# gk969/stm32-speech-recognition

Hardware: AMD Instinct MI355X
Metric: utterances/sec (256-frame, 100 templates) (higher is better)
Workload: dtype int32

## Files before the change

### stm32_speech_recognition_amd/csrc/k_mfcc.hip

```cpp
#include "sr_fft_dev.h"

#ifndef SR_MEL_CHUNKED
#define SR_MEL_CHUNKED 1
#endif

namespace sr {

constexpr int kMfccWaves = 4;
constexpr int kFramesPerWave = 16, kFramesPerWaveMid = 4, kFramesPerWaveSmall = 1;
constexpr int kMelPad = kMel + 1;
__device__ __forceinline__ constexpr int mel_chunk_word(int j) { return 256 * ((j >> 2) & 1) + 4 * ((j >> 3) ^ (4 * ((j >> 2) & 1))) + (j & 3); }
constexpr int mfcc_wave_lds_words(int fpw) { return kXchgWords + fpw * kMelPad + 64; }

template <int kFPW, typename Args = MfccArgs>
__global__ void __launch_bounds__(64 * kMfccWaves, 4) k_mfcc(const Args a)
{
    constexpr int kFeat = mfcc_feat_kind<Args>;
    constexpr uint32_t kFeatW = (kFeat == SR_FEAT_FFT || kFeat == SR_FEAT_MAG) ? kBins : kMel;
    constexpr int kWaveLdsWords = mfcc_wave_lds_words(kFPW);
    extern __shared__ __attribute__((aligned(16))) uint32_t smem[];
    __shared__ uint32_t s_dctM[kCoef * kMelPad];
    __shared__ int s_dctS[kCoef * kMelPad];
    __shared__ u32x4 s_tw3[kTw3Row * 4], s_tw5[8 * 64];
    __shared__ u32x4 s_tm[4 * 64];
    const int lane = threadIdx.x & 63, w = __builtin_amdgcn_readfirstlane(threadIdx.x >> 6);
    uint32_t *buf = smem + w * kWaveLdsWords;
    uint32_t *xw = buf;
    uint32_t *powb = buf + kXchgWords, *moff = powb + kFPW * kMelPad;

    for (int i = threadIdx.x; i < kCoef * kMel; i += blockDim.x) {
        const int c = a.t.dct[i], o = (i / kMel) * kMelPad + i % kMel;
        s_dctM[o] = (uint32_t)(((c < 0 ? -c : c) * 262144 + 99) / 100);
        s_dctS[o] = (c > 0) - (c < 0);
    }
    __syncthreads();

    LaneTw tw;
    load_lane_tw(a.t, lane, tw);
    if (w == 0 && lane < 4) {
        const uint32_t *f = &tw.s3[0][0][0];
#pragma unroll
        for (int c = 0; c < 8; c++) s_tw3[lane * kTw3Row + c] = u32x4{f[4 * c], f[4 * c + 1], f[4 * c + 2], f[4 * c + 3]};
    }
    if (w == 1 % kMfccWaves) store_tw32(s_tw5, lane, tw.s5);
#ifndef SR_INJECT_LDS_RACE
    if (w == 2 % kMfccWaves) {
#pragma unroll
        for (int c = 0; c < 2; c++) {
            s_tm[64 * c + lane] = *(const u32x4 *)(a.t.tri_even_m + 8 * lane + 4 * c);
            s_tm[64 * (c + 2) + lane] = *(const u32x4 *)(a.t.tri_odd_m + 8 * lane + 4 * c);
        }
    }
#endif
    __syncthreads();
#ifdef SR_INJECT_LDS_RACE
    if (w == 2 % kMfccWaves) {
#if SR_INJECT_LDS_RACE >= 2
        __builtin_amdgcn_s_sleep(127);
#endif
#pragma unroll
        for (int c = 0; c < 2; c++) {
            s_tm[64 * c + lane] = *(const u32x4 *)(a.t.tri_even_m + 8 * lane + 4 * c);
            s_tm[64 * (c + 2) + lane] = *(const u32x4 *)(a.t.tri_odd_m + 8 * lane + 4 * c);
        }
    }
#endif
    int hamm_m[3];
#pragma unroll
    for (int k = 0; k < 3; k++) hamm_m[k] = (lane + 64 * k < kFrameLen) ? hamm_fused_multiplier(a.t.hamm[lane + 64 * k]) : 0;
    int f_lo = 0, p_hi = 0, p_lo = 0, x_hi = 0, x_lo = 0;
    if (lane < kMel) {
        const int h = lane;
        f_lo = (h == 0) ? 0 : (int)a.t.tri_cen[h - 1];
        const int f_hi = (h == kMel - 1) ? kBins : (int)a.t.tri_cen[h + 1];
        const int ih = f_hi - 1, il = f_lo ? f_lo - 1 : 0, half = (h & 1) ? kBins : 0;
#if SR_MEL_CHUNKED
        p_hi = half + mel_chunk_word(ih), x_hi = (ih >> 3) > 0 ? (ih >> 3) - 1 : 0;
        p_lo = half + mel_chunk_word(il), x_lo = (il >> 3) > 0 ? (il >> 3) - 1 : 0;
#else
        p_hi = half + ih, x_hi = (ih >> 3) > 0 ? (ih >> 3) - 1 : 0;
        p_lo = half + il, x_lo = (il >> 3) > 0 ? (il >> 3) - 1 : 0;
#endif
    }
    const uint32_t tw_off = 32u * (uint32_t)lane;
#if SR_MEL_CHUNKED
    const int e_base = mel_chunk_word(lane);
    constexpr int kEs = 32, kEh = 128;
    const int c0 = mel_chunk_word(8 * lane), c1 = mel_chunk_word(8 * lane + 4);
#else
    const int e_base = lane;
    constexpr int kEs = 64, kEh = 256;
    const int c0 = 8 * lane, c1 = 8 * lane + 4;
#endif

    uint32_t item = blockIdx.x;
    uint32_t nx_nfrm = 0;
    int nx_mid = 0, nx_seg0 = 0;
    if (item < a.n_items) {
        const sr_vad_rec *rec = a.vad + item / a.tiles;
        nx_nfrm = rec->frm_num;
        nx_mid = (int)rec->atap.mid_val;
        nx_seg0 = rec->seg[0];
    }
    for (; item < a.n_items; item += gridDim.x) {
        const uint32_t b = item / a.tiles, tile = item - b * a.tiles;
        const uint32_t nfrm = nx_nfrm;
        const int mid = nx_mid, seg0 = nx_seg0;
        if (item + gridDim.x < a.n_items) {
            const sr_vad_rec *rec = a.vad + (item + gridDim.x) / a.tiles;
            nx_nfrm = rec->frm_num;
            nx_mid = (int)rec->atap.mid_val;
            nx_seg0 = rec->seg[0];
        }
        const uint16_t *row = a.pcm + (uint64_t)b * a.pcm_stride;
        int16_t *out = a.mfcc + (uint64_t)b * a.max_frames * kCoef;
        const uint32_t f0 = tile * (kMfccWaves * kFPW) + w * kFPW;
        uint32_t *frow = nullptr;
        if constexpr (kFeat != 0) frow = a.feat + (uint64_t)b * a.max_frames * kFeatW;
        uint32_t nf = 0;
        if (f0 < nfrm) nf = (nfrm - f0 < (uint32_t)kFPW) ? nfrm - f0 : (uint32_t)kFPW;

        uint32_t s_pp[3] = {0, 0, 0};
        if (nf) {
            const uint16_t *x = row + seg0 + (int)kHop * (int)f0;
#pragma unroll
            for (int k = 0; k < 3; k++) {
                const int i = lane + 64 * k;
                if (i < kFrameLen) s_pp[k] = *(const u32_align2 *)(x + i - 1);
            }
        }
        for (uint32_t fi = 0; fi < nf; fi++) {
#pragma unroll
            for (int k = 0; k < 3; k++) {
                const int i = lane + 64 * k;
                if (i < kFrameLen) xw[i] = k == 0 ? window_sample<4>(s_pp[k], mid, hamm_m[k]) : window_sample<2>(s_pp[k], mid, hamm_m[k]);
            }
            if (fi + 1 < nf) {
                const uint16_t *x = row + seg0 + (int)kHop * (int)(f0 + fi + 1);
#pragma unroll
                for (int k = 0; k < 3; k++) {
                    const int i = lane + 64 * k;
                    if (i < kFrameLen) s_pp[k] = *(const u32_align2 *)(x + i - 1);
                }
            }
            wave_sync();
            uint32_t v[4][4], u[4][4];
            fft_front_real160(xw, lane, tw, s_tw3, v);
            fft_exchange(buf, lane, v, u);
#pragma unroll
            for (int e4 = 0; e4 < 4; e4++)
                bfly_pk<false>(u[0][e4], u[1][e4], u[2][e4], u[3][e4], tw.s4[0][0], tw.s4[0][1], tw.s4[1][0], tw.s4[1][1],
                               tw.s4[2][0], tw.s4[2][1], tw.s4[3][0], tw.s4[3][1]);
            wave_sync();
            uint32_t k5[4][4][2];
            load_tw32(s_tw5, lane, k5);
            uint32_t nn[8];
#pragma unroll
            for (int e3 = 0; e3 < 4; e3++) {
                bfly_pk<true>(u[e3][0], u[e3][1], u[e3][2], u[e3][3], k5[e3][0][0], k5[e3][0][1], k5[e3][1][0],
                              k5[e3][1][1], k5[e3][2][0], k5[e3][2][1], k5[e3][3][0], k5[e3][3][1]);
                if constexpr (kFeat == SR_FEAT_FFT) {
                    uint32_t *fr = frow + (f0 + fi) * kFeatW + lane + 64 * e3;
                    fr[0] = u[e3][0];
                    fr[256] = u[e3][1];
                }
                nn[2 * e3] = (uint32_t)sdot2z(u[e3][0], u[e3][0]);
                nn[2 * e3 + 1] = (uint32_t)sdot2z(u[e3][1], u[e3][1]);
            }
            const uint32_t nmax = max(max(max(max(nn[0], nn[1]), nn[2]), max(max(nn[3], nn[4]), nn[5])), max(nn[6], nn[7]));
            const bool quiet = __builtin_expect(__builtin_amdgcn_ballot_w64(nmax > kMagSmallMax) == 0, 1);
            u32x4 tw_e[2], tw_o[2];
            bool cheap = true;
            if (!quiet) {
#pragma unroll
                for (int c = 0; c < 2; c++) {
                    tw_e[c] = *(const u32x4 *)((const char *)a.t.tri_even32 + tw_off + 16 * c);
                    tw_o[c] = *(const u32x4 *)((const char *)a.t.tri_odd32 + tw_off + 16 * c);
                }
                cheap = __builtin_amdgcn_ballot_w64(nmax > a.mag_cheap_max) == 0;
            } else {
                asm volatile("" : "=v"(tw_e[0]), "=v"(tw_e[1]), "=v"(tw_o[0]), "=v"(tw_o[1]));
            }
            uint32_t *eb = buf + e_base;
            if (cheap) {
#pragma unroll
                for (int e3 = 0; e3 < 4; e3++) {
                    const f32x2 m = f32x2{__builtin_amdgcn_sqrtf((float)(int)nn[2 * e3]), __builtin_amdgcn_sqrtf((float)(int)nn[2 * e3 + 1])} *
                                    f32x2{10.0f, 10.0f};
                    const uint32_t m0 = cvt_u32(m.x), m1 = cvt_u32(m.y);
                    if constexpr (kFeat == SR_FEAT_MAG) {
                        uint32_t *fr = frow + (f0 + fi) * kFeatW + lane + 64 * e3;
                        fr[0] = m0;
                        fr[256] = m1;
                    }
                    eb[kEs * e3] = umul24(m0, m0);
                    eb[kEs * e3 + kEh] = umul24(m1, m1);
                }
            } else {
#pragma unroll
                for (int e3 = 0; e3 < 4; e3++) {
                    const f32x2 m = sqrt_rn_int2(f32x2{(float)(int)nn[2 * e3], (float)(int)nn[2 * e3 + 1]}) * f32x2{10.0f, 10.0f};
                    const uint32_t m0 = cvt_u32(m.x), m1 = cvt_u32(m.y);
                    if constexpr (kFeat == SR_FEAT_MAG) {
                        uint32_t *fr = frow + (f0 + fi) * kFeatW + lane + 64 * e3;
                        fr[0] = m0;
                        fr[256] = m1;
                    }
                    eb[kEs * e3] = umul24(m0, m0);
                    eb[kEs * e3 + kEh] = umul24(m1, m1);
                }
            }
            wave_sync();
            uint32_t pe[8], po[8], xe, xo;
            {
                const uint4 q0 = *(const uint4 *)(buf + c0), q1 = *(const uint4 *)(buf + c1);
                const uint32_t e[8] = {q0.x, q0.y, q0.z, q0.w, q1.x, q1.y, q1.z, q1.w};
                uint32_t se = 0, so = 0;
                if (quiet) {
#pragma unroll
                    for (int c = 0; c < 2; c++) {
                        const u32x4 me = s_tm[64 * c + lane], mo = s_tm[64 * (c + 2) + lane];
#pragma unroll
                        for (int k = 0; k < 4; k++) {
                            const uint32_t es = e[4 * c + k] << 4;
                            se += mel_term_fused(es, me[k]);
                            so += mel_term_fused(es, mo[k]);
                            pe[4 * c + k] = se;
                            po[4 * c + k] = so;
                        }
                    }
                } else {
#pragma unroll
                    for (int c = 0; c < 2; c++) {
#pragma unroll
                        for (int k = 0; k < 4; k++) {
                            se += e[4 * c + k] * tw_e[c][k] / 100u;
                            so += e[4 * c + k] * tw_o[c][k] / 100u;
                            pe[4 * c + k] = se;
                            po[4 * c + k] = so;
                        }
                    }
                }
                xe = wave_scan_incl(se);
                xo = wave_scan_incl(so);
            }
            *(uint4 *)(buf + c0) = make_uint4(pe[0], pe[1], pe[2], pe[3]);
            *(uint4 *)(buf + c1) = make_uint4(pe[4], pe[5], pe[6], pe[7]);
            *(uint4 *)(buf + kBins + c0) = make_uint4(po[0], po[1], po[2], po[3]);
            *(uint4 *)(buf + kBins + c1) = make_uint4(po[4], po[5], po[6], po[7]);
            buf[2 * kBins + lane] = xe;
            moff[lane] = xo;
            wave_sync();
            if (lane < kMel) {
                const uint32_t *X = (lane & 1) ? moff : buf + 2 * kBins;
                const uint32_t hi = buf[p_hi] + X[x_hi], lo = f_lo ? buf[p_lo] + X[x_lo] : 0u;
                powb[fi * kMelPad + lane] = hi - lo;
                if constexpr (kFeat == SR_FEAT_MEL) frow[(f0 + fi) * kFeatW + lane] = hi - lo;
            }
            wave_sync();
        }

        {
            constexpr int kLogRounds = (kFPW * kMelPad + 63) / 64;
            const uint32_t n_log = nf * kMelPad;
            uint32_t nv[kLogRounds], mv[kLogRounds];
            u32x2 tv[kLogRounds];
#pragma unroll
            for (int r = 0; r < kLogRounds; r++) {
                const uint32_t t = lane + 64u * r;
                nv[r] = powb[t];
                mv[r] = log100_est(nv[r]);
                tv[r] = *(const u32_pair_align4 *)((const char *)a.t.log_thr + 4u * mv[r]);
            }
#pragma unroll
            for (int r = 0; r < kLogRounds; r++) {
                const uint32_t t = lane + 64u * r;
                if (t < n_log) powb[t] = log100_fix(nv[r], mv[r], tv[r].x, tv[r].y) << 14;
            }
        }
        wave_sync();
        if constexpr (kFeat == SR_FEAT_LOGMEL) {
            uint32_t *fw = frow + f0 * kFeatW;
            for (uint32_t t = lane; t < nf * kFeatW; t += 64) {
                const uint32_t fi = t / kFeatW, h = t - fi * kFeatW;
                fw[t] = powb[fi * kMelPad + h] >> 14;
            }
        }
        {
            int16_t *out_w = out + (size_t)f0 * kCoef;
#pragma unroll
            for (uint32_t t = lane; t < (uint32_t)(kFPW * kCoef); t += 64) {
                if (t < nf * kCoef) {
                    const uint32_t fi = umul24(t, 10923u) >> 17, h = t - umul24(fi, (uint32_t)kCoef);
                    const uint32_t *pw = powb + umul24(fi, (uint32_t)kMelPad), *dm = s_dctM + umul24(h, (uint32_t)kMelPad);
                    const int *ds = s_dctS + umul24(h, (uint32_t)kMelPad);
                    int acc = 0;
#pragma unroll
                    for (int i = 0; i < kMel; i++) acc = mad24((int)__umulhi(pw[i], dm[i]), ds[i], acc);
                    out_w[t] = (int16_t)acc;
                }
            }
        }
        wave_sync();
        {
            const uint32_t r0 = f0 + nf, r1 = (f0 + kFPW < a.max_frames) ? f0 + kFPW : a.max_frames;
            for (uint32_t t = r0 * kCoef + lane; t < r1 * kCoef && r0 < r1; t += 64) out[t] = 0;
        }
        if constexpr (kFeat != 0) {
            const uint32_t r0 = f0 + nf, r1 = (f0 + kFPW < a.max_frames) ? f0 + kFPW : a.max_frames;
            for (uint32_t t = r0 * kFeatW + lane; t < r1 * kFeatW && r0 < r1; t += 64) frow[t] = 0;
        }
    }
}

uint32_t mfcc_ext_frames_per_tile();
int mfcc_ext_occupancy(int *per_cu);
void launch_mfcc_ext(const MfccArgs &a, uint32_t grid, hipStream_t s);
void launch_mfcc_ext_features(const MfccArgs &a, int kind, uint32_t *feat, uint32_t grid, hipStream_t s);

uint32_t mfcc_frames_per_tile(uint32_t frame_len) { return frame_len == 320 ? mfcc_ext_frames_per_tile() : (uint32_t)(kMfccWaves * kFramesPerWave); }
uint32_t mfcc_frames_per_tile_small(uint32_t frame_len, uint32_t which)
{
    return frame_len == 320 ? mfcc_ext_frames_per_tile() : (uint32_t)(kMfccWaves * (which ? kFramesPerWaveSmall : kFramesPerWaveMid));
}

uint32_t mfcc_resident_workgroups(uint32_t frame_len)
{
    int dev = 0, n_cu = 0, per_cu = 0;
    if (hipGetDevice(&dev) != hipSuccess) return 0;
    if (hipDeviceGetAttribute(&n_cu, hipDeviceAttributeMultiprocessorCount, dev) != hipSuccess || n_cu < 1) return 0;
    int e;
    if (frame_len == 320)
        e = mfcc_ext_occupancy(&per_cu);
    else
        e = (int)hipOccupancyMaxActiveBlocksPerMultiprocessor(&per_cu, k_mfcc<kFramesPerWave>, 64 * kMfccWaves,
                                                              (size_t)kMfccWaves * mfcc_wave_lds_words(kFramesPerWave) * sizeof(uint32_t));
    if (e != (int)hipSuccess || per_cu < 1) return 0;
    return (uint32_t)(per_cu * n_cu);
}

void launch_mfcc(const MfccArgs &a, hipStream_t s)
{
    if (a.generic) {
        launch_mfcc_gen(a, s);
        return;
    }
    if (a.n_items == 0) return;
    const uint32_t cap = a.grid_cap ? a.grid_cap : 4096u;
    const uint32_t grid = a.n_items < cap ? a.n_items : cap;
    if (a.frame_len == 320) {
        launch_mfcc_ext(a, grid, s);
        return;
    }
    if (a.small_tiles == 2) {
        const size_t lds = (size_t)kMfccWaves * mfcc_wave_lds_words(kFramesPerWaveSmall) * sizeof(uint32_t);
        hipLaunchKernelGGL(k_mfcc<kFramesPerWaveSmall>, dim3(grid), dim3(64 * kMfccWaves), lds, s, a);
        return;
    }
    if (a.small_tiles == 1) {
        const size_t lds = (size_t)kMfccWaves * mfcc_wave_lds_words(kFramesPerWaveMid) * sizeof(uint32_t);
        hipLaunchKernelGGL(k_mfcc<kFramesPerWaveMid>, dim3(grid), dim3(64 * kMfccWaves), lds, s, a);
        return;
    }
    const size_t lds = (size_t)kMfccWaves * mfcc_wave_lds_words(kFramesPerWave) * sizeof(uint32_t);
    hipLaunchKernelGGL(k_mfcc<kFramesPerWave>, dim3(grid), dim3(64 * kMfccWaves), lds, s, a);
}

template <int kFPW, int kKind>
static void launch_mfcc_feat_kind(const MfccArgs &a, uint32_t *feat, uint32_t grid, hipStream_t s)
{
    const size_t lds = (size_t)kMfccWaves * mfcc_wave_lds_words(kFPW) * sizeof(uint32_t);
    hipLaunchKernelGGL((k_mfcc<kFPW, MfccFeatArgs<kKind>>), dim3(grid), dim3(64 * kMfccWaves), lds, s, mfcc_feat_args<kKind>(a, feat));
}
template <int kFPW>
static void launch_mfcc_feat_form(const MfccArgs &a, int kind, uint32_t *feat, uint32_t grid, hipStream_t s)
{
    switch (kind) {
    case SR_FEAT_FFT: launch_mfcc_feat_kind<kFPW, SR_FEAT_FFT>(a, feat, grid, s); break;
    case SR_FEAT_MAG: launch_mfcc_feat_kind<kFPW, SR_FEAT_MAG>(a, feat, grid, s); break;
    case SR_FEAT_MEL: launch_mfcc_feat_kind<kFPW, SR_FEAT_MEL>(a, feat, grid, s); break;
    case SR_FEAT_LOGMEL: launch_mfcc_feat_kind<kFPW, SR_FEAT_LOGMEL>(a, feat, grid, s); break;
    default: break;
    }
}

void launch_mfcc_features(const MfccArgs &a, int kind, uint32_t *feat, hipStream_t s)
{
    if (a.generic) {
        launch_mfcc_gen_features(a, kind, feat, s);
        return;
    }
    if (a.n_items == 0) return;
    const uint32_t cap = a.grid_cap ? a.grid_cap : 4096u;
    const uint32_t grid = a.n_items < cap ? a.n_items : cap;
    if (a.frame_len == 320)
        launch_mfcc_ext_features(a, kind, feat, grid, s);
    else if (a.small_tiles == 2)
        launch_mfcc_feat_form<kFramesPerWaveSmall>(a, kind, feat, grid, s);
    else if (a.small_tiles == 1)
        launch_mfcc_feat_form<kFramesPerWaveMid>(a, kind, feat, grid, s);
    else
        launch_mfcc_feat_form<kFramesPerWave>(a, kind, feat, grid, s);
}

}
```

### stm32_speech_recognition_amd/csrc/sr_dev.h

```cpp
#pragma once
#include <cstdlib>

#include "sr_device.h"
#include "sr_tables.h"

namespace sr {

typedef short short2v __attribute__((ext_vector_type(2)));
typedef uint32_t u32x2 __attribute__((ext_vector_type(2)));
typedef uint32_t u32x4 __attribute__((ext_vector_type(4)));

__device__ __forceinline__ int sdot2(uint32_t a, uint32_t b, int c)
{
    return __builtin_amdgcn_sdot2(__builtin_bit_cast(short2v, a), __builtin_bit_cast(short2v, b), c, false);
}
__device__ __forceinline__ int sext_lo(uint32_t w) { return (int)(short)(w & 0xFFFFu); }
__device__ __forceinline__ int sext_hi(uint32_t w) { return (int)w >> 16; }
__device__ __forceinline__ uint32_t pack16(int re, int im) { return ((uint32_t)re & 0xFFFFu) | ((uint32_t)im << 16); }

__device__ __forceinline__ int sdot2z(uint32_t a, uint32_t b)
{
    int r;
    asm("v_dot2_i32_i16 %0, %1, %2, 0" : "=v"(r) : "v"(a), "v"(b));
    return r;
}
__device__ __forceinline__ int sdot2a(uint32_t a, uint32_t b, int c)
{
    int r;
    asm("v_dot2_i32_i16 %0, %1, %2, %3" : "=v"(r) : "v"(a), "v"(b), "v"(c));
    return r;
}
__device__ __forceinline__ int preemph95(int p) { return (int)((float)p * 0.95000005f); }
__device__ __forceinline__ int neg_preemph95(int p) { return (int)((float)p * -0.95000005f); }
__device__ __forceinline__ int window_quotient(int c, int nq, int hm)
{
    int u;
    asm("v_add_lshl_u32 %0, %1, %2, %3" : "=v"(u) : "v"(c), "v"(nq), "n"(kWinShift));
    const long long P = (long long)u * (long long)hm + (long long)(unsigned long long)(uint32_t)(u >> 31);
    return (int)(P >> 32);
}
template <int SH = 2>
__device__ __forceinline__ uint32_t window_sample(uint32_t prev_cur, int mid, int hm)
{
    const int nq = neg_preemph95((int)(prev_cur & 0xFFFFu) - mid);
    const int c = (int)(prev_cur >> 16) - mid;
    int u;
    asm("v_add_lshl_u32 %0, %1, %2, %3" : "=v"(u) : "v"(c), "v"(nq), "n"(kWinShift));
    const long long P = (long long)u * (long long)hm + (long long)(unsigned long long)(uint32_t)(u >> 31);
    int r;
    asm("v_bfe_i32 %0, %1, %2, %3" : "=v"(r) : "v"((int)(P >> 32)), "n"(SH), "n"(16 - SH));
    return (uint32_t)r;
}
__device__ __forceinline__ int mul24(int a, int b) { return __mul24(a, b); }
__device__ __forceinline__ uint32_t umul24(uint32_t a, uint32_t b) { return __umul24(a, b); }
__device__ __forceinline__ int mad24(int a, int b, int c)
{
    int r;
    asm("v_mad_i32_i24 %0, %1, %2, %3" : "=v"(r) : "v"(a), "v"(b), "v"(c));
    return r;
}

__device__ __forceinline__ uint32_t mel_term_fused(uint32_t e_shl4, uint32_t m) { return __umulhi(e_shl4, m); }
__device__ __forceinline__ uint32_t mel_tri_of_multiplier(uint32_t m) { return __umulhi(m, 1600u); }

__device__ __forceinline__ float sqrt_rn_int(float f)
{
    const float y = __builtin_amdgcn_rsqf(f);
    const float s0 = f * y, h = 0.5f * y;
    const float r = __builtin_fmaf(-s0, s0, f);
    return __builtin_fmaf(r, h, s0);
}

__device__ __forceinline__ uint32_t mag10_small(float f)
{
    uint32_t r;
    const float m = __builtin_amdgcn_sqrtf(f) * 10.0f;
    asm("v_cvt_u32_f32 %0, %1" : "=v"(r) : "v"(m));
    return r;
}

__device__ __forceinline__ uint32_t cvt_u32(float x)
{
    uint32_t r;
    asm("v_cvt_u32_f32 %0, %1" : "=v"(r) : "v"(x));
    return r;
}
typedef float f32x2 __attribute__((ext_vector_type(2)));
__device__ __forceinline__ f32x2 sqrt_rn_int2(f32x2 f)
{
    const f32x2 y = {__builtin_amdgcn_rsqf(f.x), __builtin_amdgcn_rsqf(f.y)};
    const f32x2 s0 = f * y, h = f32x2{0.5f, 0.5f} * y;
    const f32x2 r = __builtin_elementwise_fma(-s0, s0, f);
    return __builtin_elementwise_fma(r, h, s0);
}
typedef uint32_t u32_align2 __attribute__((aligned(2)));
typedef uint32_t u32x2_raw __attribute__((ext_vector_type(2)));
typedef u32x2_raw u32_pair_align4 __attribute__((aligned(4)));
typedef uint32_t u32x2_align2 __attribute__((ext_vector_type(2), aligned(2)));

typedef unsigned short u16x2 __attribute__((ext_vector_type(2)));
__device__ __forceinline__ uint32_t pk_add(uint32_t a, uint32_t b)
{
    return __builtin_bit_cast(uint32_t, (u16x2)(__builtin_bit_cast(u16x2, a) + __builtin_bit_cast(u16x2, b)));
}
__device__ __forceinline__ uint32_t pk_sub(uint32_t a, uint32_t b)
{
    return __builtin_bit_cast(uint32_t, (u16x2)(__builtin_bit_cast(u16x2, a) - __builtin_bit_cast(u16x2, b)));
}
__device__ __forceinline__ uint32_t pk_ashr(uint32_t a, int n)
{
    return __builtin_bit_cast(uint32_t, (short2v)(__builtin_bit_cast(short2v, a) >> (short2v){(short)n, (short)n}));
}
__device__ __forceinline__ uint32_t pk_lshr(uint32_t a, int n)
{
    return __builtin_bit_cast(uint32_t, (u16x2)(__builtin_bit_cast(u16x2, a) >> (u16x2){(unsigned short)n, (unsigned short)n}));
}
__device__ __forceinline__ uint32_t pk_mad(uint32_t a, uint32_t c, uint32_t b)
{
    return __builtin_bit_cast(uint32_t, (u16x2)(__builtin_bit_cast(u16x2, a) * __builtin_bit_cast(u16x2, c) +
                                                __builtin_bit_cast(u16x2, b)));
}
__device__ __forceinline__ uint32_t pk_mad_swap(uint32_t a, uint32_t c, uint32_t b)
{
    uint32_t r;
    asm("v_pk_mad_u16 %0, %1, %2, %3 op_sel:[1,0,0] op_sel_hi:[0,1,1]" : "=v"(r) : "v"(a), "s"(c), "v"(b));
    return r;
}
__device__ __forceinline__ uint32_t pk_hi16(int lo_src, int hi_src)
{
    return __builtin_amdgcn_perm((uint32_t)hi_src, (uint32_t)lo_src, 0x07060302u);
}
__device__ __forceinline__ uint32_t pk_s15(int lo_src, int hi_src)
{
    uint32_t r = (uint32_t)lo_src >> 15;
    asm("v_lshrrev_b32_sdwa %0, %1, %2 dst_sel:WORD_1 dst_unused:UNUSED_PRESERVE src0_sel:DWORD src1_sel:DWORD\n\ts_nop 0"
        : "+v"(r)
        : "v"(15), "v"(hi_src));
    return r;
}

__device__ __forceinline__ void wave_sync()
{
    __builtin_amdgcn_fence(__ATOMIC_RELEASE, "wavefront");
    __builtin_amdgcn_wave_barrier();
    __builtin_amdgcn_fence(__ATOMIC_ACQUIRE, "wavefront");
}

__device__ __forceinline__ uint32_t wave_sum(uint32_t v)
{
#pragma unroll
    for (int d = 32; d >= 1; d >>= 1) v += __shfl_xor(v, d, 64);
    return v;
}
__device__ __forceinline__ uint32_t wave_min_u32(uint32_t v)
{
#pragma unroll
    for (int d = 32; d >= 1; d >>= 1) {
        uint32_t o = __shfl_xor(v, d, 64);
        v = o < v ? o : v;
    }
    return v;
}
__device__ __forceinline__ uint32_t wave_max(uint32_t v)
{
#pragma unroll
    for (int d = 32; d >= 1; d >>= 1) {
        uint32_t o = __shfl_xor(v, d, 64);
        v = o > v ? o : v;
    }
    return v;
}

template <int CTRL, int ROW_MASK>
__device__ __forceinline__ uint32_t dpp_take(uint32_t v)
{
    return (uint32_t)__builtin_amdgcn_update_dpp(0, (int)v, CTRL, ROW_MASK, 0xF, false);
}
__device__ __forceinline__ uint32_t wave_scan_incl(uint32_t v)
{
    v += dpp_take<0x111, 0xF>(v);
    v += dpp_take<0x112, 0xF>(v);
    v += dpp_take<0x114, 0xF>(v);
    v += dpp_take<0x118, 0xF>(v);
    asm("s_nop 1\n\tv_add_u32_dpp %0, %0, %0 row_bcast:15 row_mask:0xa" : "+v"(v));
    asm("s_nop 1\n\tv_add_u32_dpp %0, %0, %0 row_bcast:31 row_mask:0xc" : "+v"(v));
    return v;
}

__device__ __forceinline__ uint32_t log100_est(uint32_t n)
{
    return (uint32_t)(int)__builtin_amdgcn_fmed3f(__log2f((float)n) * 69.31471806f, 1.0f, (float)(kLogMax - 1));
}
__device__ __forceinline__ uint32_t log100_fix(uint32_t n, uint32_t m, uint32_t t0, uint32_t t1)
{
    return (uint32_t)((int)m - (int)(n < t0) + (int)(n >= t1));
}
__device__ __forceinline__ uint32_t log100_u32(uint32_t n, const uint32_t *__restrict__ thr)
{
    const uint32_t m = log100_est(n);
    return log100_fix(n, m, thr[m], thr[m + 1]);
}

}
```

Measured before the change: 3.172 million.

## Process frame pairs per wave, sharing overlapping PCM loads and pre-emphasis

For the 16-frames-per-wave variant, the loop now handles two consecutive frames per iteration. One set of global loads covers both frames' overlapping sample window. Pre-emphasis is computed once and staged through LDS, and each frame gets its own Hamming multiply. This cuts redundant global loads and pre-emphasis work for overlapping frames, at the cost of extra LDS traffic, a wave sync and more register pressure.

Result: no change. 3.183 million, median of 6 (+0.3%).

```diff
diff --git a/stm32_speech_recognition_amd/csrc/k_mfcc.hip b/stm32_speech_recognition_amd/csrc/k_mfcc.hip
--- a/stm32_speech_recognition_amd/csrc/k_mfcc.hip
+++ b/stm32_speech_recognition_amd/csrc/k_mfcc.hip
@@ -11,6 +11,10 @@
 constexpr int kMelPad = kMel + 1;
 __device__ __forceinline__ constexpr int mel_chunk_word(int j) { return 256 * ((j >> 2) & 1) + 4 * ((j >> 3) ^ (4 * ((j >> 2) & 1))) + (j & 3); }
 constexpr int mfcc_wave_lds_words(int fpw) { return kXchgWords + fpw * kMelPad + 64; }
+__device__ __forceinline__ bool pair_row_has(int k, int lane, bool two)
+{
+    return k < 2 || (k == 2 && (two || lane < kFrameLen - 128)) || (k == 3 && two && lane < kFrameLen + kHop - 192);
+}
 
 template <int kFPW, typename Args = MfccArgs>
 __global__ void __launch_bounds__(64 * kMfccWaves, 4) k_mfcc(const Args a)
@@ -68,6 +72,12 @@
     int hamm_m[3];
 #pragma unroll
     for (int k = 0; k < 3; k++) hamm_m[k] = (lane + 64 * k < kFrameLen) ? hamm_fused_multiplier(a.t.hamm[lane + 64 * k]) : 0;
+    constexpr bool kPair = kFPW == kFramesPerWave;
+    constexpr uint32_t kStep = kPair ? 2 : 1;
+    constexpr int kRows = kPair ? 4 : 3;
+    const int hamm_m2 = kPair ? hamm_fused_multiplier(a.t.hamm[128 + (lane & 31)]) : 0;
+    uint32_t *tpre = buf + 576 - kHop;
+    const int t2 = 128 + lane + (lane >= 32 ? kHop - 32 : 0);
     int f_lo = 0, p_hi = 0, p_lo = 0, x_hi = 0, x_lo = 0;
     if (lane < kMel) {
         const int h = lane;
@@ -120,144 +130,177 @@
         uint32_t nf = 0;
         if (f0 < nfrm) nf = (nfrm - f0 < (uint32_t)kFPW) ? nfrm - f0 : (uint32_t)kFPW;
 
-        uint32_t s_pp[3] = {0, 0, 0};
+        uint32_t s_pp[kRows] = {};
         if (nf) {
             const uint16_t *x = row + seg0 + (int)kHop * (int)f0;
-#pragma unroll
-            for (int k = 0; k < 3; k++) {
-                const int i = lane + 64 * k;
-                if (i < kFrameLen) s_pp[k] = *(const u32_align2 *)(x + i - 1);
-            }
-        }
-        for (uint32_t fi = 0; fi < nf; fi++) {
-#pragma unroll
-            for (int k = 0; k < 3; k++) {
-                const int i = lane + 64 * k;
-                if (i < kFrameLen) xw[i] = k == 0 ? window_sample<4>(s_pp[k], mid, hamm_m[k]) : window_sample<2>(s_pp[k], mid, hamm_m[k]);
-            }
-            if (fi + 1 < nf) {
-                const uint16_t *x = row + seg0 + (int)kHop * (int)(f0 + fi + 1);
+            const bool two = kPair && nf > 1;
+#pragma unroll
+            for (int k = 0; k < kRows; k++)
+                if (pair_row_has(k, lane, two)) s_pp[k] = *(const u32_align2 *)(x + lane + 64 * k - 1);
+        }
+        uint32_t hb0 = 0, hb1 = 0, h2 = 0;
+        for (uint32_t fi = 0; fi < nf; fi += kStep) {
+            if constexpr (kPair) {
+                int u[kRows];
+#pragma unroll
+                for (int k = 0; k < kRows; k++) u[k] = window_pre(s_pp[k], mid);
+#pragma unroll
+                for (int k = 1; k < kRows; k++) tpre[64 * k + lane] = (uint32_t)u[k];
+                xw[lane] = window_hamm<4>(u[0], hamm_m[0]);
+                xw[64 + lane] = window_hamm<2>(u[1], hamm_m[1]);
+                if (fi + 2 < nf) {
+                    const uint16_t *x = row + seg0 + (int)kHop * (int)(f0 + fi + 2);
+                    const bool two = fi + 3 < nf;
+#pragma unroll
+                    for (int k = 0; k < kRows; k++)
+                        if (pair_row_has(k, lane, two)) s_pp[k] = *(const u32_align2 *)(x + lane + 64 * k - 1);
+                }
+                wave_sync();
+                h2 = window_hamm<2>((int)tpre[t2], hamm_m2);
+                if (lane < 32) xw[128 + lane] = h2;
+                hb0 = window_hamm<4>((int)tpre[kHop + lane], hamm_m[0]);
+                hb1 = window_hamm<2>((int)tpre[kHop + 64 + lane], hamm_m[1]);
+            } else {
 #pragma unroll
                 for (int k = 0; k < 3; k++) {
                     const int i = lane + 64 * k;
-                    if (i < kFrameLen) s_pp[k] = *(const u32_align2 *)(x + i - 1);
+                    if (i < kFrameLen) xw[i] = k == 0 ? window_sample<4>(s_pp[k], mid, hamm_m[k]) : window_sample<2>(s_pp[k], mid, hamm_m[k]);
+                }
+                if (fi + 1 < nf) {
+                    const uint16_t *x = row + seg0 + (int)kHop * (int)(f0 + fi + 1);
+#pragma unroll
+                    for (int k = 0; k < 3; k++) {
+                        const int i = lane + 64 * k;
+                        if (i < kFrameLen) s_pp[k] = *(const u32_align2 *)(x + i - 1);
+                    }
                 }
             }
             wave_sync();
-            uint32_t v[4][4], u[4][4];
-            fft_front_real160(xw, lane, tw, s_tw3, v);
-            fft_exchange(buf, lane, v, u);
-#pragma unroll
-            for (int e4 = 0; e4 < 4; e4++)
-                bfly_pk<false>(u[0][e4], u[1][e4], u[2][e4], u[3][e4], tw.s4[0][0], tw.s4[0][1], tw.s4[1][0], tw.s4[1][1],
-                               tw.s4[2][0], tw.s4[2][1], tw.s4[3][0], tw.s4[3][1]);
-            wave_sync();
-            uint32_t k5[4][4][2];
-            load_tw32(s_tw5, lane, k5);
-            uint32_t nn[8];
-#pragma unroll
-            for (int e3 = 0; e3 < 4; e3++) {
-                bfly_pk<true>(u[e3][0], u[e3][1], u[e3][2], u[e3][3], k5[e3][0][0], k5[e3][0][1], k5[e3][1][0],
-                              k5[e3][1][1], k5[e3][2][0], k5[e3][2][1], k5[e3][3][0], k5[e3][3][1]);
-                if constexpr (kFeat == SR_FEAT_FFT) {
-                    uint32_t *fr = frow + (f0 + fi) * kFeatW + lane + 64 * e3;
-                    fr[0] = u[e3][0];
-                    fr[256] = u[e3][1];
-                }
-                nn[2 * e3] = (uint32_t)sdot2z(u[e3][0], u[e3][0]);
-                nn[2 * e3 + 1] = (uint32_t)sdot2z(u[e3][1], u[e3][1]);
-            }
-            const uint32_t nmax = max(max(max(max(nn[0], nn[1]), nn[2]), max(max(nn[3], nn[4]), nn[5])), max(nn[6], nn[7]));
-            const bool quiet = __builtin_expect(__builtin_amdgcn_ballot_w64(nmax > kMagSmallMax) == 0, 1);
-            u32x4 tw_e[2], tw_o[2];
-            bool cheap = true;
-            if (!quiet) {
-#pragma unroll
-                for (int c = 0; c < 2; c++) {
-                    tw_e[c] = *(const u32x4 *)((const char *)a.t.tri_even32 + tw_off + 16 * c);
-                    tw_o[c] = *(const u32x4 *)((const char *)a.t.tri_odd32 + tw_off + 16 * c);
-                }
-                cheap = __builtin_amdgcn_ballot_w64(nmax > a.mag_cheap_max) == 0;
-            } else {
-                asm volatile("" : "=v"(tw_e[0]), "=v"(tw_e[1]), "=v"(tw_o[0]), "=v"(tw_o[1]));
-            }
-            uint32_t *eb = buf + e_base;
-            if (cheap) {
+#pragma unroll
+            for (uint32_t s = 0; s < kStep; s++) {
+                const uint32_t fc = fi + s;
+                if (s == 1) {
+                    if (fc >= nf) break;
+                    xw[lane] = hb0;
+                    xw[64 + lane] = hb1;
+                    if (lane >= 32) xw[96 + lane] = h2;
+                    wave_sync();
+                }
+                uint32_t v[4][4], u[4][4];
+                fft_front_real160(xw, lane, tw, s_tw3, v);
+                fft_exchange(buf, lane, v, u);
+#pragma unroll
+                for (int e4 = 0; e4 < 4; e4++)
+                    bfly_pk<false>(u[0][e4], u[1][e4], u[2][e4], u[3][e4], tw.s4[0][0], tw.s4[0][1], tw.s4[1][0], tw.s4[1][1],
+                                   tw.s4[2][0], tw.s4[2][1], tw.s4[3][0], tw.s4[3][1]);
+                wave_sync();
+                uint32_t k5[4][4][2];
+                load_tw32(s_tw5, lane, k5);
+                uint32_t nn[8];
 #pragma unroll
                 for (int e3 = 0; e3 < 4; e3++) {
-                    const f32x2 m = f32x2{__builtin_amdgcn_sqrtf((float)(int)nn[2 * e3]), __builtin_amdgcn_sqrtf((float)(int)nn[2 * e3 + 1])} *
-                                    f32x2{10.0f, 10.0f};
-                    const uint32_t m0 = cvt_u32(m.x), m1 = cvt_u32(m.y);
-                    if constexpr (kFeat == SR_FEAT_MAG) {
-                        uint32_t *fr = frow + (f0 + fi) * kFeatW + lane + 64 * e3;
-                        fr[0] = m0;
-                        fr[256] = m1;
-                    }
-                    eb[kEs * e3] = umul24(m0, m0);
-                    eb[kEs * e3 + kEh] = umul24(m1, m1);
-                }
-            } else {
-#pragma unroll
-                for (int e3 = 0; e3 < 4; e3++) {
-                    const f32x2 m = sqrt_rn_int2(f32x2{(float)(int)nn[2 * e3], (float)(int)nn[2 * e3 + 1]}) * f32x2{10.0f, 10.0f};
-                    const uint32_t m0 = cvt_u32(m.x), m1 = cvt_u32(m.y);
-                    if constexpr (kFeat == SR_FEAT_MAG) {
-                        uint32_t *fr = frow + (f0 + fi) * kFeatW + lane + 64 * e3;
-                        fr[0] = m0;
-                        fr[256] = m1;
-                    }
-                    eb[kEs * e3] = umul24(m0, m0);
-                    eb[kEs * e3 + kEh] = umul24(m1, m1);
-                }
-            }
-            wave_sync();
-            uint32_t pe[8], po[8], xe, xo;
-            {
-                const uint4 q0 = *(const uint4 *)(buf + c0), q1 = *(const uint4 *)(buf + c1);
-                const uint32_t e[8] = {q0.x, q0.y, q0.z, q0.w, q1.x, q1.y, q1.z, q1.w};
-                uint32_t se = 0, so = 0;
-                if (quiet) {
+                    bfly_pk<true>(u[e3][0], u[e3][1], u[e3][2], u[e3][3], k5[e3][0][0], k5[e3][0][1], k5[e3][1][0],
+                                  k5[e3][1][1], k5[e3][2][0], k5[e3][2][1], k5[e3][3][0], k5[e3][3][1]);
+                    if constexpr (kFeat == SR_FEAT_FFT) {
+                        uint32_t *fr = frow + (f0 + fc) * kFeatW + lane + 64 * e3;
+                        fr[0] = u[e3][0];
+                        fr[256] = u[e3][1];
+                    }
+                    nn[2 * e3] = (uint32_t)sdot2z(u[e3][0], u[e3][0]);
+                    nn[2 * e3 + 1] = (uint32_t)sdot2z(u[e3][1], u[e3][1]);
+                }
+                const uint32_t nmax = max(max(max(max(nn[0], nn[1]), nn[2]), max(max(nn[3], nn[4]), nn[5])), max(nn[6], nn[7]));
+                const bool quiet = __builtin_expect(__builtin_amdgcn_ballot_w64(nmax > kMagSmallMax) == 0, 1);
+                u32x4 tw_e[2], tw_o[2];
+                bool cheap = true;
+                if (!quiet) {
 #pragma unroll
                     for (int c = 0; c < 2; c++) {
-                        const u32x4 me = s_tm[64 * c + lane], mo = s_tm[64 * (c + 2) + lane];
-#pragma unroll
-                        for (int k = 0; k < 4; k++) {
-                            const uint32_t es = e[4 * c + k] << 4;
-                            se += mel_term_fused(es, me[k]);
-                            so += mel_term_fused(es, mo[k]);
-                            pe[4 * c + k] = se;
-                            po[4 * c + k] = so;
+                        tw_e[c] = *(const u32x4 *)((const char *)a.t.tri_even32 + tw_off + 16 * c);
+                        tw_o[c] = *(const u32x4 *)((const char *)a.t.tri_odd32 + tw_off + 16 * c);
+                    }
+                    cheap = __builtin_amdgcn_ballot_w64(nmax > a.mag_cheap_max) == 0;
+                } else {
+                    asm volatile("" : "=v"(tw_e[0]), "=v"(tw_e[1]), "=v"(tw_o[0]), "=v"(tw_o[1]));
+                }
+                uint32_t *eb = buf + e_base;
+                if (cheap) {
+#pragma unroll
+                    for (int e3 = 0; e3 < 4; e3++) {
+                        const f32x2 m = f32x2{__builtin_amdgcn_sqrtf((float)(int)nn[2 * e3]), __builtin_amdgcn_sqrtf((float)(int)nn[2 * e3 + 1])} *
+                                        f32x2{10.0f, 10.0f};
+                        const uint32_t m0 = cvt_u32(m.x), m1 = cvt_u32(m.y);
+                        if constexpr (kFeat == SR_FEAT_MAG) {
+                            uint32_t *fr = frow + (f0 + fc) * kFeatW + lane + 64 * e3;
+                            fr[0] = m0;
+                            fr[256] = m1;
                         }
+                        eb[kEs * e3] = umul24(m0, m0);
+                        eb[kEs * e3 + kEh] = umul24(m1, m1);
                     }
                 } else {
 #pragma unroll
-                    for (int c = 0; c < 2; c++) {
-#pragma unroll
-                        for (int k = 0; k < 4; k++) {
-                            se += e[4 * c + k] * tw_e[c][k] / 100u;
-                            so += e[4 * c + k] * tw_o[c][k] / 100u;
-                            pe[4 * c + k] = se;
-                            po[4 * c + k] = so;
+                    for (int e3 = 0; e3 < 4; e3++) {
+                        const f32x2 m = sqrt_rn_int2(f32x2{(float)(int)nn[2 * e3], (float)(int)nn[2 * e3 + 1]}) * f32x2{10.0f, 10.0f};
+                        const uint32_t m0 = cvt_u32(m.x), m1 = cvt_u32(m.y);
+                        if constexpr (kFeat == SR_FEAT_MAG) {
+                            uint32_t *fr = frow + (f0 + fc) * kFeatW + lane + 64 * e3;
+                            fr[0] = m0;
+                            fr[256] = m1;
                         }
-                    }
-                }
-                xe = wave_scan_incl(se);
-                xo = wave_scan_incl(so);
-            }
-            *(uint4 *)(buf + c0) = make_uint4(pe[0], pe[1], pe[2], pe[3]);
-            *(uint4 *)(buf + c1) = make_uint4(pe[4], pe[5], pe[6], pe[7]);
-            *(uint4 *)(buf + kBins + c0) = make_uint4(po[0], po[1], po[2], po[3]);
-            *(uint4 *)(buf + kBins + c1) = make_uint4(po[4], po[5], po[6], po[7]);
-            buf[2 * kBins + lane] = xe;
-            moff[lane] = xo;
-            wave_sync();
-            if (lane < kMel) {
-                const uint32_t *X = (lane & 1) ? moff : buf + 2 * kBins;
-                const uint32_t hi = buf[p_hi] + X[x_hi], lo = f_lo ? buf[p_lo] + X[x_lo] : 0u;
-                powb[fi * kMelPad + lane] = hi - lo;
-                if constexpr (kFeat == SR_FEAT_MEL) frow[(f0 + fi) * kFeatW + lane] = hi - lo;
-            }
-            wave_sync();
+                        eb[kEs * e3] = umul24(m0, m0);
+                        eb[kEs * e3 + kEh] = umul24(m1, m1);
+                    }
+                }
+                wave_sync();
+                uint32_t pe[8], po[8], xe, xo;
+                {
+                    const uint4 q0 = *(const uint4 *)(buf + c0), q1 = *(const uint4 *)(buf + c1);
+                    const uint32_t e[8] = {q0.x, q0.y, q0.z, q0.w, q1.x, q1.y, q1.z, q1.w};
+                    uint32_t se = 0, so = 0;
+                    if (quiet) {
+#pragma unroll
+                        for (int c = 0; c < 2; c++) {
+                            const u32x4 me = s_tm[64 * c + lane], mo = s_tm[64 * (c + 2) + lane];
+#pragma unroll
+                            for (int k = 0; k < 4; k++) {
+                                const uint32_t es = e[4 * c + k] << 4;
+                                se += mel_term_fused(es, me[k]);
+                                so += mel_term_fused(es, mo[k]);
+                                pe[4 * c + k] = se;
+                                po[4 * c + k] = so;
+                            }
+                        }
+                    } else {
+#pragma unroll
+                        for (int c = 0; c < 2; c++) {
+#pragma unroll
+                            for (int k = 0; k < 4; k++) {
+                                se += e[4 * c + k] * tw_e[c][k] / 100u;
+                                so += e[4 * c + k] * tw_o[c][k] / 100u;
+                                pe[4 * c + k] = se;
+                                po[4 * c + k] = so;
+                            }
+                        }
+                    }
+                    xe = wave_scan_incl(se);
+                    xo = wave_scan_incl(so);
+                }
+                *(uint4 *)(buf + c0) = make_uint4(pe[0], pe[1], pe[2], pe[3]);
+                *(uint4 *)(buf + c1) = make_uint4(pe[4], pe[5], pe[6], pe[7]);
+                *(uint4 *)(buf + kBins + c0) = make_uint4(po[0], po[1], po[2], po[3]);
+                *(uint4 *)(buf + kBins + c1) = make_uint4(po[4], po[5], po[6], po[7]);
+                buf[2 * kBins + lane] = xe;
+                moff[lane] = xo;
+                wave_sync();
+                if (lane < kMel) {
+                    const uint32_t *X = (lane & 1) ? moff : buf + 2 * kBins;
+                    const uint32_t hi = buf[p_hi] + X[x_hi], lo = f_lo ? buf[p_lo] + X[x_lo] : 0u;
+                    powb[fc * kMelPad + lane] = hi - lo;
+                    if constexpr (kFeat == SR_FEAT_MEL) frow[(f0 + fc) * kFeatW + lane] = hi - lo;
+                }
+                wave_sync();
+            }
         }
 
         {
diff --git a/stm32_speech_recognition_amd/csrc/sr_dev.h b/stm32_speech_recognition_amd/csrc/sr_dev.h
--- a/stm32_speech_recognition_amd/csrc/sr_dev.h
+++ b/stm32_speech_recognition_amd/csrc/sr_dev.h
@@ -39,17 +39,26 @@
     const long long P = (long long)u * (long long)hm + (long long)(unsigned long long)(uint32_t)(u >> 31);
     return (int)(P >> 32);
 }
-template <int SH = 2>
-__device__ __forceinline__ uint32_t window_sample(uint32_t prev_cur, int mid, int hm)
+__device__ __forceinline__ int window_pre(uint32_t prev_cur, int mid)
 {
     const int nq = neg_preemph95((int)(prev_cur & 0xFFFFu) - mid);
     const int c = (int)(prev_cur >> 16) - mid;
     int u;
     asm("v_add_lshl_u32 %0, %1, %2, %3" : "=v"(u) : "v"(c), "v"(nq), "n"(kWinShift));
+    return u;
+}
+template <int SH = 2>
+__device__ __forceinline__ uint32_t window_hamm(int u, int hm)
+{
     const long long P = (long long)u * (long long)hm + (long long)(unsigned long long)(uint32_t)(u >> 31);
     int r;
     asm("v_bfe_i32 %0, %1, %2, %3" : "=v"(r) : "v"((int)(P >> 32)), "n"(SH), "n"(16 - SH));
     return (uint32_t)r;
+}
+template <int SH = 2>
+__device__ __forceinline__ uint32_t window_sample(uint32_t prev_cur, int mid, int hm)
+{
+    return window_hamm<SH>(window_pre(prev_cur, mid), hm);
 }
 __device__ __forceinline__ int mul24(int a, int b) { return __mul24(a, b); }
 __device__ __forceinline__ uint32_t umul24(uint32_t a, uint32_t b) { return __umul24(a, b); }
```
